# MartinMikkelsen/TensorTrainNumerics.jl

Hardware: AMD Instinct MI355X
Metric: TT cores/sec for QTT Laplacian apply+round, d=30 rank-64 (higher is better)
Workload: dtype f64

## Files before the change

### tensortrainnumerics.jl_amd/csrc/ttn_dense_kernels.h

```cpp
#pragma once
#include "ttn_wg_prims.h"
#include "ttn_wg_gemm.h"
#include "ttn_wg_lq.h"
#include "ttn_wg_jacobi.h"
#include "ttn_wg_chol.h"

struct CompressArgs {
    TTDev tt;
    long long max_bond;
    double truncerr;
    int sweeps;
    int k_single;
    int k_first, k_last;
    double* scratch;
    long long scratch_stride;
    int pmax, qmax;
    double* sv_out;
    int sv_steps;
    int* status;
    int* sweep_stats;
    int fast;
    int fused;
    TTODev op;
    TTDev x;
// ... 739 lines not shown
            for (int kk = wave; kk < half; kk += TTN_NWAVES) {
                int i, j;
                if (kk == 0) { i = round; j = pe - 1; }
                else { i = (round + kk) % (pe - 1); j = (round + pe - 1 - kk) % (pe - 1); }
                if (i > j) { const int t = i; i = j; j = t; }
                if (j >= p) continue;
                lds_f64* xi = Ms + i * LDQ;
                lds_f64* xj = Ms + j * LDQ;
                double u[4], v[4];
                double a = 0.0, b_ = 0.0, g = 0.0;
#pragma unroll
                for (int t4 = 0; t4 < 4; ++t4) {
                    const int c = lane + 64 * t4;
                    u[t4] = (c < q) ? xi[c] : 0.0; v[t4] = (c < q) ? xj[c] : 0.0;
                    a = fma(u[t4], u[t4], a); b_ = fma(v[t4], v[t4], b_); g = fma(u[t4], v[t4], g);
                }
                a = wave_sum(a); b_ = wave_sum(b_); g = wave_sum(g);
                if (a <= aneg || b_ <= aneg) continue;
                if (g * g <= tol2 * a * b_) continue;
                const double dd = b_ - a, hh = g + g;
                const double hyp = __builtin_amdgcn_sqrt(fma(dd, dd, hh * hh));
                const double t = copysign(hh * __builtin_amdgcn_rcp(fabs(dd) + hyp), hh * dd);
                const double cs = fast_rsqrt2(fma(t, t, 1.0)), sn = cs * t;
#pragma unroll
                for (int t4 = 0; t4 < 4; ++t4) {
                    const int c = lane + 64 * t4;
                    if (c < q) { xi[c] = cs * u[t4] - sn * v[t4]; xj[c] = sn * u[t4] + cs * v[t4]; }
                }
                if (lane < p) { const double u = Es[i * 17 + lane], v = Es[j * 17 + lane]; Es[i * 17 + lane] = cs * u - sn * v; Es[j * 17 + lane] = sn * u + cs * v; }
                rotated = 1;
            }
            __syncthreads();
        }
        if (rotated && lane == 0) atomicOr((int*)flg, 1);
        __syncthreads();
        conv = !(*flg);
        __syncthreads();
    }
    for (int i = wave; i < p; i += TTN_NWAVES) {
        double a = 0.0;
        for (int j = lane; j < q; j += 64) { const double v = Ms[i * LDQ + j]; a = fma(v, v, a); }
        a = wave_sum(a);
        if (lane == 0) nr[i] = sqrt(a);
    }
    __syncthreads();
    for (int c = tid; c < p; c += TTN_WG) {
        const double sc = nr[c];
        int pos = 0;
        for (int j = 0; j < p; ++j) { const double sj = nr[j]; pos += (sj > sc) || (sj == sc && j < c); }
        Q.perm[pos] = c;
        Q.sigs[pos] = sc;
    }
    __syncthreads();
    const int r = wg_rank_rule_core(Q.rank_rule, Q.truncerr, Q.max_bond, Q.sigs, Q.iflag, p, p, s0);
    if (Q.sv_row)
        for (int i = tid; i < Q.pmax; i += TTN_WG) Q.sv_row[i] = (i < p) ? Q.sigs[i] * s0 : -1.0;
    const View Lfv = mkview(ck, Idx{Dl, (long long)n1, 1}, plain((long long)n1 * Dl));
    const View Rfv = mkview(ck1, plain(n2), Idx{n2, 1, (long long)n2 * r});
    const View Lo = wide ? Lfv : tview(Rfv);
    const View Ro = wide ? Rfv : tview(Lfv);
    const double sq0 = sqrt(s0);
    for (int e = tid; e < p * r; e += TTN_WG) {
        const int row = e % p, j = e / p;
        const double sj = Q.sigs[j];
        const int pj = Q.perm[j];
        const bool keep = (sj > 0.0) && (sj * sj > aneg);
        Lo.p[ix(Lo.r, row) + ix(Lo.c, j)] = keep ? Es[pj * 17 + row] * (sq0 * sqrt(sj)) : 0.0;
    }
    for (int e = tid; e < r * q; e += TTN_WG) {
        const int col = e % q, j = e / q;
        const double sj = Q.sigs[j];
        const int pj = Q.perm[j];
        const bool keep = (sj > 0.0) && (sj * sj > aneg);
        Ro.p[ix(Ro.r, j) + ix(Ro.c, col)] = keep ? Ms[pj * LDQ + col] * (sq0 / sqrt(sj)) : 0.0;
    }
    if (tid == 0) { *rank_out = r; if (!conv) *Q.status_b = TTN_ST_JACOBI; }
    __syncthreads();
    return sweeps;
}

__device__ int wg_eig128(const double* Gg, double* Vst, int r, int nev, double* sig, double* lds, int* iwork, double* dwork);
__device__ int wg_eig64(const double* Gg, int ldg, double* Vst, int r, int nev, double* sig, double* lds, int* iwork, double* dwork);

struct BondIO {
    double *ck, *ck1;
    int n1, n2, Dl, rm, Dr;
    long long* rank_out;
    int cap;
};
template <int SWAP>
__device__ __forceinline__ void wg_bond_step_io(const CompressArgs& P, int b, const BondIO& io, int k, int step, double* lds, bool virt) {
    const int tid = threadIdx.x;
    const int n1 = io.n1, n2 = io.n2;
    const int Dl = io.Dl, rm = io.rm, Dr = io.Dr;
    const int mr = n1 * Dl, mc = n2 * Dr;
    double* ck = io.ck;
    double* ck1 = io.ck1;
    const View Am = mkview(ck, Idx{Dl, (long long)n1, 1}, plain((long long)n1 * Dl));
    const View Bm = mkview(ck1, plain(n2), Idx{n2, 1, (long long)n2 * rm});
    const bool wide = mr <= mc;
    const int p = wide ? mr : mc, q = wide ? mc : mr;
    const View Ap = wide ? Am : tview(Bm);
    const View Bp = wide ? Bm : tview(Am);

    BondCtx S;
    S.ldsX = lds;
    S.red = lds + GEMM_LDS_TOTAL;
    S.Ts = S.red + 32;
    S.Ss = S.Ts + QR_NB * QR_NB;
    S.taus = S.Ss + QR_NB * QR_NB;
    S.scal = S.taus + QR_NB;
    S.iflag = reinterpret_cast<int*>(S.scal + 8);
    S.nrm2 = S.scal + 16;
    double* scr = P.scratch + (long long)blockIdx.x * P.scratch_stride;
    const long long pq = (long long)P.pmax * P.qmax;
    S.M = scr;
    S.M2 = S.M + pq;
    S.Vb = S.M2 + pq;
    S.Wb = S.Vb + (long long)QR_NB * P.qmax;
    S.Us = S.Wb + (long long)P.pmax * QR_NB;
    S.Xg = S.Us + (long long)P.pmax * P.pmax;
    S.sig = S.Xg + (long long)P.pmax * P.pmax;
    S.sigs = S.sig + P.pmax;
    S.perm = reinterpret_cast<int*>(S.sigs + P.pmax);
    S.Ga = S.sigs + 2 * P.pmax;
    S.Gb = S.Ga + 128 * 128;
    S.Cc = S.Gb + 128 * 128;
    S.T1 = S.Cc + 128 * 128;
    S.T2 = S.T1 + 128 * 128;
    S.T3 = S.T2 + 128 * 128;
    if (pq >= 3 * 128 * 128) {
        S.Ga = S.M2; S.Gb = S.M2 + 128 * 128; S.T2 = S.M2 + 2 * 128 * 128;
    }

    bool virt_live = false;
    if (virt) {
        if (wide && rm >= p) virt_live = true;
        else wg_materialize_core(P, b, k + 1);
    }

    const View Lfv = mkview(ck, Idx{Dl, (long long)n1, 1}, plain((long long)n1 * Dl));
    int nsw_total = 0;
    bool done = false;

    if (SWAP == 0 && P.fast && rm < p && rm <= TTN_LDS_COLS && rm >= 2) {
        double sa = 0.0, sb = 0.0;
        sa = wg_absmax(ck, (long long)n1 * Dl * rm, S.red);
        sb = wg_absmax(ck1, (long long)n2 * rm * Dr, S.red);
        bool ok = (sa > 0.0) && (sb > 0.0);
        const double sA = wide ? sa : sb, sB = wide ? sb : sa;
        const double s0 = sA * sB;
        const View Gav = mkview(S.Ga, plain(1), plain(128));
        const View Gbv = mkview(S.Gb, plain(1), plain(128));
        const View Ccv = mkview(S.Cc, plain(1), plain(128));
        bool diagA = false;
        if (ok) {
            wg_syrk2(rm, p, tview(Ap), Gav, 1.0 / (sA * sA), rm, q, Bp, Gbv, 1.0 / (sB * sB), lds);
            if (rm == 64 && !(P.fast & 4) && !(P.fast & 8)) {
                const double wmax = wg_diag_test_t3(S.Ga, S.Gb, S.T3, S.Ss, S.red);
                diagA = wmax <= FAST_DIAG_TOL;
            }
            if (diagA) {
            } else if (rm <= TTN_LDS_COLS / 2) {
                for (int e = tid; e < rm * 128; e += TTN_WG) if ((e & 127) < rm) { S.ldsX[e] = S.Ga[e]; S.ldsX[TTN_LDS_IMG / 2 + e] = S.Gb[e]; }
                __syncthreads();
                ok = wg_chol2_lds128(rm, S.ldsX, S.Ts, S.iflag, S.scal + 1) == 0;
                for (int e = tid; e < rm * 128; e += TTN_WG) if ((e & 127) < rm) { S.Ga[e] = S.ldsX[e]; S.Gb[e] = S.ldsX[TTN_LDS_IMG / 2 + e]; }
                __syncthreads();
            } else {
                for (int e = tid; e < rm * 128; e += TTN_WG) if ((e & 127) < rm) S.ldsX[e] = S.Ga[e];
                __syncthreads();
                ok = wg_chol_lds128(rm, S.ldsX, S.red, S.iflag, S.scal + 1) == 0;
                for (int e = tid; e < rm * 128; e += TTN_WG) if ((e & 127) < rm) S.Ga[e] = S.ldsX[e];
                __syncthreads();
                if (ok) {
                    for (int e = tid; e < rm * 128; e += TTN_WG) if ((e & 127) < rm) S.ldsX[e] = S.Gb[e];
                    __syncthreads();
                    ok = wg_chol_lds128(rm, S.ldsX, S.red, S.iflag, S.scal + 1) == 0;
                    for (int e = tid; e < rm * 128; e += TTN_WG) if ((e & 127) < rm) S.Gb[e] = S.ldsX[e];
                    __syncthreads();
                }
            }
        }
        int r = 0, rk = 0;
        if (ok) {
            int nsw = 1;
            if (diagA) {
                ok = wg_eig64(S.T3, 128, S.T2, 64, 64, S.sigs, lds, reinterpret_cast<int*>(S.Ts), S.Ts + 64) == 0;
                for (int j = tid; j < 64; j += TTN_WG) S.perm[j] = j;
                if (tid == 0) S.scal[0] = 64.0 * DBL_EPSILON * DBL_EPSILON * S.sigs[0] * S.sigs[0];
                __syncthreads();
            } else {
            wg_gemm(rm, rm, rm, tview(Gav), Gbv, Ccv, 1.0, 0.0, lds);
            if (rm == 64 && !(P.fast & 4)) {
                wg_gemm(64, 64, 64, Ccv, tview(Ccv), mkview(S.T3, plain(1), plain(128)), 1.0, 0.0, lds);
                ok = wg_eig64(S.T3, 128, S.T2, 64, 64, S.sigs, lds, reinterpret_cast<int*>(S.Ts), S.Ts + 64) == 0;
                for (int j = tid; j < 64; j += TTN_WG) S.perm[j] = j;
                if (tid == 0) S.scal[0] = 64.0 * DBL_EPSILON * DBL_EPSILON * S.sigs[0] * S.sigs[0];
                __syncthreads();
            } else {
                for (int e = tid; e < rm * 128; e += TTN_WG) { const int c = e >> 7, r_ = e & 127; S.ldsX[e] = (r_ < rm) ? S.Cc[c * 128 + r_] : 0.0; }
                __syncthreads();
                nsw = uni32(wg_svd_cols(P, S, rm, S.ldsX, 128, true));
                nsw_total += (nsw < 0 ? -nsw : nsw);
            }
            }
            ok = ok && (nsw > 0) && (S.sigs[rm - 1] * FAST_KAPPA_MAX >= S.sigs[0]) && (S.sigs[rm - 1] * S.sigs[rm - 1] > S.scal[0]);
        }
        if (ok) {
            r = wg_rank_rule(P, S, rm, p, s0);
            rk = r < rm ? r : rm;
            const double fa = sqrt(s0) / sA, fb = sqrt(s0) / sB;
            if (diagA) {
                wg_scale_t12_diag(S.ldsX, S.sigs, S.perm, S.Ga, S.T1, S.T2, rk, fa, fb, S.Ts);
            } else {
                for (int e = tid; e < rm * rk; e += TTN_WG) {
                    const int row = e % rm, j = e / rm;
                    const double sj = S.sigs[j], xv = S.ldsX[S.perm[j] * 128 + row];
                    const double rs = sqrt(sj);
                    S.T1[j * 128 + row] = xv * (fa / (sj * sj * rs));
                    S.T2[j * 128 + row] = xv * (fb / (sj * rs));
                }
                __syncthreads();
            }
            const View T1v = mkview(S.T1, plain(1), plain(128));
            const View T2v = mkview(S.T2, plain(1), plain(128));
            double* LfT = S.M;
            double* RfT = S.M + (long long)p * rk;
            const View Lft = mkview(LfT, plain(1), plain(p));
            const View Rft = mkview(RfT, plain(q), plain(1));
            if (diagA) {
                wg_gemm_ra2(rk, p, rm, tview(T1v), tview(Ap), tview(Lft), 1.0, rk, q, rm, tview(T2v), Bp, Rft, 1.0, lds);
            } else {
            wg_gemm(rm, rk, rm, tview(Ccv), T1v, mkview(S.T3, plain(1), plain(128)), 1.0, 0.0, lds);
            wg_gemm(rm, rk, rm, Gbv, mkview(S.T3, plain(1), plain(128)), T1v, 1.0, 0.0, lds);
            wg_gemm(p, rk, rm, Ap, T1v, Lft, 1.0, 0.0, lds);
            wg_gemm(rm, rk, rm, Gav, T2v, mkview(S.T3, plain(1), plain(128)), 1.0, 0.0, lds);
            wg_gemm(rk, q, rm, tview(mkview(S.T3, plain(1), plain(128))), Bp, Rft, 1.0, 0.0, lds);
            }
            wg_syrk2(rk, p, tview(Lft), mkview(S.T1, plain(1), plain(128)), 1.0, rk, q, Rft, mkview(S.T2, plain(1), plain(128)), 1.0, lds);
            ok = wg_check_diag_tab2(S.sigs, S.T1, S.T2, 128, rk, s0, S.Ts, S.red) <= FAST_CHECK_TOL;
            if (ok) {
                if (P.sv_out && step < P.sv_steps) {
                    double* so = P.sv_out + ((long long)b * P.sv_steps + step) * P.pmax;
                    for (int i = tid; i < P.pmax; i += TTN_WG) so[i] = (i < rm) ? S.sigs[i] * s0 : (i < p ? 0.0 : -1.0);
                }
                const View Rfv = mkview(ck1, plain(n2), Idx{n2, 1, (long long)n2 * r});
                const View Lo = wide ? Lfv : tview(Rfv);
                const View Ro = wide ? Rfv : tview(Lfv);
                __syncthreads();
                wg_copy_to_view(Lo, LfT, p, r, 1, p, rk, 1);
                wg_copy_to_view(Ro, RfT, r, q, q, 1, rk, 0);
                if (tid == 0) *io.rank_out = r;
                __syncthreads();
                done = true;
            }
        }
    }

    if (!done) {
        const View Mv = mkview(S.M, plain(q), plain(1));
        bool merged = false;
        if (virt_live) {
            merged = wg_fused_merge(P, b, k, p, q, Am, S.M, S.M2, pq, lds, S.scal + 6, S.red);
            if (!merged) wg_materialize_core(P, b, k + 1);
        }
        double mx_swap = 0.0;
        if (SWAP != 0) {
            for (int sA = 0; sA < n1; ++sA)
                for (int sB = 0; sB < n2; ++sB) {
                    const View Av = mkview(ck + sA, plain(n1), plain((long long)n1 * Dl));
                    const View Bv = mkview(ck1 + sB, plain(n2), plain((long long)n2 * rm));
                    if (wide) wg_gemm(Dl, Dr, rm, Av, Bv, mkview(S.M + (long long)Dl * sB * q + sA, plain(q), plain(n1)), 1.0, 0.0, lds, S.scal + 6);
                    else wg_gemm(Dr, Dl, rm, tview(Bv), tview(Av), mkview(S.M + (long long)sA * q + (long long)Dl * sB, plain((long long)n1 * q), plain(1)), 1.0, 0.0, lds, S.scal + 6);
                    mx_swap = fmax(mx_swap, unif64(S.scal[6]));
                    __syncthreads();
                }
        } else if (!merged) wg_gemm(p, q, rm, Ap, Bp, Mv, 1.0, 0.0, lds, S.scal + 6);
        const double mx = (SWAP != 0) ? mx_swap : unif64(S.scal[6]);
        const double s0 = (mx > 0.0) ? mx : 1.0;
        const double inv_s0 = 1.0 / s0;
        const bool need_lq = q > p;
        const bool x_in_lds = p <= TTN_LDS_COLS;
        double* X = x_in_lds ? S.ldsX : S.Xg;
        int ldx = x_in_lds ? 128 : p;

        const bool lq_in_lds = (long long)p * q <= GEMM_LDS_DOUBLES || GEMM_LDS_DOUBLES / p >= 2 * p;
        const bool eig_ok = SWAP == 0 && P.fast && !(P.fast & 2) && need_lq && ((p > 64 && p <= 128 && P.max_bond <= 64) || (p == 64 && P.max_bond < 64));
        const bool cholqr_ok = SWAP == 0 && P.fast && need_lq && x_in_lds && p >= 16 && p <= 64 && (long long)p * q > GEMM_LDS_DOUBLES;
        for (int attempt = (SWAP == 0 && P.fast && need_lq && (eig_ok || cholqr_ok || (x_in_lds && !lq_in_lds)) && p >= 2) ? 1 : 2; attempt <= 2 && !done; ++attempt) {
            bool ok = true;
            bool use_eig = false;
            bool cholqr = false;
            double gram_trace = 0.0;
            X = (x_in_lds || attempt == 1) ? S.ldsX : S.Xg;
            ldx = (x_in_lds || attempt == 1) ? 128 : p;
            if (attempt == 1) {
                wg_syrk(p, q, Mv, mkview(S.Ga, plain(1), plain(128)), inv_s0 * inv_s0, lds);
                use_eig = eig_ok;
                if (use_eig) {
                    if (p > 64 && p < 128) {
                        for (int e = tid; e < 128 * 128; e += TTN_WG)
                            if ((e & 127) >= p || (e >> 7) >= p) S.Ga[e] = 0.0;
                        __syncthreads();
                    }
                    const int r0 = (int)P.max_bond;
                    const int nev = (P.truncerr > 0.0 || (P.sv_out && step < P.sv_steps)) ? p : r0;
                    { double t_ = 0.0; for (int i = tid; i < p; i += TTN_WG) t_ += S.Ga[i * 129]; gram_trace = unif64(wg_sum(t_, S.red)); }
                    ok = ((p == 64) ? wg_eig64(S.Ga, 128, S.Gb, r0, nev, S.sigs, lds, reinterpret_cast<int*>(S.Ts), S.Ts + 64)
                                    : wg_eig128(S.Ga, S.Gb, r0, nev, S.sigs, lds, reinterpret_cast<int*>(S.Ts), S.Ts + 64)) == 0;
                    for (int j = tid; j < p; j += TTN_WG) { S.perm[j] = j; if (j >= nev) S.sigs[j] = 0.0; }
                    if (tid == 0) S.scal[0] = (double)p * DBL_EPSILON * DBL_EPSILON * S.sigs[0] * S.sigs[0];
                    __syncthreads();
                } else {
                wg_img_load(S.ldsX, 0, S.Ga, p, S.red);
                ok = wg_chol_lds128(p, S.ldsX, S.red, S.iflag, S.scal + 1) == 0;
                if (ok && (P.truncerr > 0.0 || (long long)p <= P.max_bond)) {
                    if (cholqr_ok) { if (unif64(S.scal[1]) <= CHOLQR_PIVOT_MAX) cholqr = true; else ok = false; }
                    else if (unif64(S.scal[1]) > FAST_KAPPA_MAX * FAST_KAPPA_MAX) ok = false;
                }
                if (cholqr) {
                    for (int e = tid; e < p * p; e += TTN_WG) { const int i = e % p, j = e / p; S.T1[i + 128 * j] = S.ldsX[i + 128 * j]; }
                    wg_trsm_lower_cols(p, q, S.ldsX, S.M, q, inv_s0, S.M2, q);
                    const View Q1v = mkview(S.M2, plain(q), plain(1));
                    wg_syrk(p, q, Q1v, mkview(S.Cc, plain(1), plain(128)), 1.0, lds);
                    const double dev = wg_img_load(S.ldsX, 0, S.Cc, p, S.red);
                    ok = dev <= CHOLQR_ORTH_MAX && wg_chol_lds128(p, S.ldsX, S.red, S.iflag, S.scal + 1) == 0;
                    if (ok) {
                        wg_img_load(S.ldsX, 64, S.T1, p, S.red);
                        wg_tril_mul_lds(p, S.ldsX);
                    }
                }
                for (int e = tid; e < p * 128; e += TTN_WG) if ((e & 127) >= p) S.ldsX[e] = 0.0;
                __syncthreads();
                }
            } else {
                if (need_lq) {
                    wg_copy_scale(S.M2, S.M, (long long)p * q, inv_s0);
                    __syncthreads();
                    wg_lq_blocked(p, q, S.M2, q, S.Vb, S.Wb, nullptr, nullptr, lds, S.Ts, S.Ss, S.taus, S.red);
                }
                const double* Lsrc = need_lq ? S.M2 : S.M;
                if (need_lq && x_in_lds) {
// ... 59 lines not shown
                    wg_gemm_ra(r, q, p, mkview(S.Us, plain(p), plain(1)), Mv, mkview(S.M2, plain(q), plain(1)), inv_s0, lds);
                    for (int e = tid; e < r * 128; e += TTN_WG) { const int c = e & 127, j = e >> 7; S.ldsX[e] = (c < q) ? S.M2[(long long)j * q + c] : 0.0; }
                    __syncthreads();
                    const int nsp = uni32(wg_svd_cols(P, S, r, S.ldsX, 128, true, q));
                    nsw_total += (nsp < 0 ? -nsp : nsp);
                    if (nsp <= 0) continue;
                    const View Rfv = mkview(ck1, plain(n2), Idx{n2, 1, (long long)n2 * r});
                    const View Lo = wide ? Lfv : tview(Rfv);
                    const View Ro = wide ? Rfv : tview(Lfv);
                    const double sq0 = sqrt(s0), aneg = S.scal[0];
                    for (int e = tid; e < r * q; e += TTN_WG) {
                        const int col = e % q, j = e / q;
                        const double sj = S.sigs[j], xv = S.ldsX[S.perm[j] * 128 + col];
                        const bool keep = (sj > 0.0) && (sj * sj > aneg);
                        Ro.p[ix(Ro.r, j) + ix(Ro.c, col)] = keep ? xv * (sq0 / sqrt(sj)) : 0.0;
                        S.M2[(long long)j * q + col] = keep ? xv * (sq0 / (sj * sqrt(sj))) : 0.0;
                    }
                    __syncthreads();
                    wg_gemm(p, r, q, Mv, mkview(S.M2, plain(1), plain(q)), Lo, inv_s0, 0.0, lds);
                    if (P.sv_out && step < P.sv_steps) {
                        double* so = P.sv_out + ((long long)b * P.sv_steps + step) * P.pmax;
                        for (int i = tid; i < P.pmax; i += TTN_WG) so[i] = (i < p) ? S.sigs[i] * s0 : -1.0;
                    }
                    if (tid == 0) *io.rank_out = r;
                    __syncthreads();
                    done = true;
                    continue;
                }
            }
            if (attempt == 2 && P.sv_out && step < P.sv_steps) {
                double* so = P.sv_out + ((long long)b * P.sv_steps + step) * P.pmax;
                for (int i = tid; i < P.pmax; i += TTN_WG) so[i] = (i < p) ? S.sigs[i] * s0 : -1.0;
            }
            const View Rfv = mkview(ck1, plain(n2), Idx{n2, 1, (long long)n2 * r});
            const View Lo = wide ? Lfv : tview(Rfv);
            const View Ro = wide ? Rfv : tview(Lfv);
            const double sq0 = sqrt(s0);
            const double aneg = S.scal[0];
            if (p <= 128 && r <= 128) {
                wg_scale_image(X, ldx, (x_in_lds || attempt == 1) ? 1 : 0, S.sigs, S.perm, Lo, S.Us, p, r, s0, aneg, (SWAP == 0) ? 0 : (wide ? 1 : 2), S.Ts);
            } else {
            for (int e = tid; e < p * r; e += TTN_WG) {
                const int row = e % p, j = e / p;
                const double sj = S.sigs[j];
                const double xv = X[(long long)S.perm[j] * ldx + row];
                const bool keep = (sj > 0.0) && (sj * sj > aneg);
                double lf, us;
                if (SWAP == 0) { lf = keep ? xv * (sq0 / sqrt(sj)) : 0.0; us = keep ? xv * (sq0 / (sj * sqrt(sj))) : 0.0; }
                else if (wide) { lf = keep ? xv / sj : 0.0; us = keep ? xv * (s0 / sj) : 0.0; }
                else { lf = keep ? xv * s0 : 0.0; us = keep ? xv / (sj * sj) : 0.0; }
                Lo.p[ix(Lo.r, row) + ix(Lo.c, j)] = lf;
                S.Us[(long long)j * p + row] = us;
            }
            }
            __syncthreads();
            wg_gemm_ra(r, q, p, mkview(S.Us, plain(p), plain(1)), Mv, Ro, inv_s0, lds);
            if (attempt == 1) {
                wg_syrk(r, q, Ro, mkview(S.T2, plain(1), plain(128)), 1.0, lds);
                const double e2 = (r <= 128) ? wg_check_diag_tab(S.sigs, S.T2, 128, r, s0, S.Ts, S.red) : unif64(wg_check_diag(S, S.T2, 128, r, s0));
                if (!(e2 <= (cholqr ? CHOLQR_CHECK_TOL : FAST_CHECK_TOL))) continue;
                if (P.sv_out && step < P.sv_steps) {
                    double* so = P.sv_out + ((long long)b * P.sv_steps + step) * P.pmax;
                    for (int i = tid; i < P.pmax; i += TTN_WG) so[i] = (i < p) ? S.sigs[i] * s0 : -1.0;
                }
            }
            if (tid == 0) *io.rank_out = r;
            __syncthreads();
            done = true;
        }
    }
    if (tid == 0) P.sweep_stats[b] += nsw_total;
    __syncthreads();
}

__device__ __forceinline__ void wg_bond_step(const CompressArgs& P, int b, int k, int step, double* lds, bool virt = false ) {
    const TTDev& T = P.tt;
    long long* rks = T.rks + (long long)b * (T.d + 1);
    BondIO io;
    io.n1 = uni32(T.dims[k]); io.n2 = uni32(T.dims[k + 1]);
    io.Dl = uni32((int)rks[k]); io.rm = uni32((int)rks[k + 1]); io.Dr = uni32((int)rks[k + 2]);
    io.ck = T.data + (long long)b * T.stride + T.off[k];
    io.ck1 = T.data + (long long)b * T.stride + T.off[k + 1];
    io.rank_out = rks + k + 1;
    {
        const int mr = io.n1 * io.Dl, mc = io.n2 * io.Dr;
        const int p = mr <= mc ? mr : mc, q = mr <= mc ? mc : mr;
        if (P.fast && p >= 2 && p <= SMALL_STEP_PMAX && q <= SMALL_STEP_QMAX && P.pmax >= p) {
            if (virt) wg_materialize_core(P, b, k + 1);
            SmallStepArgs Q;
            Q.truncerr = P.truncerr; Q.max_bond = P.max_bond; Q.rank_rule = P.rank_rule; Q.pmax = P.pmax;
            Q.sv_row = (P.sv_out && step < P.sv_steps) ? P.sv_out + ((long long)b * P.sv_steps + step) * P.pmax : nullptr;
            Q.status_b = P.status + b;
            Q.red = lds + GEMM_LDS_TOTAL;
            Q.scal = Q.red + 32 + 2 * QR_NB * QR_NB + QR_NB;
            Q.iflag = reinterpret_cast<int*>(Q.scal + 8);
            double* scr = P.scratch + (long long)blockIdx.x * P.scratch_stride;
            const long long pq = (long long)P.pmax * P.qmax;
            double* sig = scr + 2 * pq + (long long)QR_NB * P.qmax + (long long)P.pmax * QR_NB + 2LL * P.pmax * P.pmax;
            Q.sigs = sig + P.pmax;
            Q.perm = reinterpret_cast<int*>(Q.sigs + P.pmax);
            const int nsw = wg_bond_small(Q, io.ck, io.ck1, io.n1, io.n2, io.Dl, io.rm, io.Dr, io.rank_out, lds);
            if (threadIdx.x == 0) P.sweep_stats[b] += nsw;
            __syncthreads();
            return;
        }
    }
    wg_bond_step_io<0>(P, b, io, k, step, lds, virt);
}

__global__ void TTN_KERNEL_BOUNDS k_compress(CompressArgs P) {
    TTN_SETPRIO_BASE();
    extern __shared__ double lds[];
    const int d = P.tt.d;
    const int per_sweep = 2 * (d - 1);
    const int nsteps = (P.k_single > 0) ? 1 : (P.k_single < 0) ? ((P.k_first <= P.k_last ? P.k_last - P.k_first : P.k_first - P.k_last) + 1)
                                                               : P.sweeps * per_sweep;
    int b = blockIdx.x;
    while (b < P.tt.batch) {
        if (threadIdx.x == 0) P.sweep_stats[b] = 0;
        __syncthreads();
        if (P.fused && !(P.k_single < 0 && P.fused_first_real)) wg_materialize_core(P, b, (P.k_single < 0) ? P.k_first : 0);
        for (int step = 0; step < nsteps; ++step) {
            int k;
            bool virt = false;
            if (P.k_single > 0) k = P.k_single - 1;
            else if (P.k_single < 0) { k = (P.k_first <= P.k_last) ? P.k_first + step : P.k_first - step; virt = P.fused != 0; }
            else {
                const int i = step % per_sweep;
                k = (i < d - 1) ? i : per_sweep - 1 - i;
                virt = P.fused && step < d - 1;
            }
            wg_bond_step(P, b, k, step, lds, virt);
        }
        if (!P.next_train) break;
        int* nb = reinterpret_cast<int*>(lds + GEMM_LDS_TOTAL);
        if (threadIdx.x == 0) *nb = (int)gridDim.x + atomicAdd(P.next_train, 1);
        __syncthreads();
        b = uni32(*nb);
        __syncthreads();
    }
}
```

### tensortrainnumerics.jl_amd/csrc/ttn_wg_gemm.h

```cpp
#pragma once
#include "ttn_wg_prims.h"

#define GEMM_BK 16
#define GEMM_LD 145
#define GEMM_LDS_DOUBLES (TTN_LDS_IMG + 512)


struct GemmDesc {
    int m, n, k, pad;
    View A, B, C;
    double alpha, beta;
    unsigned long long* amax;
};
#if TTN_WG == 512
#define GEMM_TAB_ENTRIES 704
#define GEMM_KSLAB 512
#define GEMM_SMALL_KMAX 256
#else
#define GEMM_TAB_ENTRIES 1536
#define GEMM_KSLAB 768
#define GEMM_SMALL_KMAX 512
#endif
#define GEMM_DESC_DOUBLES (32 + GEMM_TAB_ENTRIES)
#define GEMM_LDS_TOTAL (GEMM_LDS_DOUBLES + GEMM_DESC_DOUBLES)
// ... 418 lines not shown
                const int kk = (K0) + fx + 16 * u;                                                                      \
                co_[u] = colT[kk < q ? kk : 0];                                                                         \
            }                                                                                                           \
            _Pragma("unroll") for (int j = 0; j < JMAX; ++j) {                                                           \
                const int row = sy + RG * j;                                                                            \
                _Pragma("unroll") for (int u = 0; u < KC16; ++u) {                                                       \
                    const int kk = (K0) + fx + 16 * u;                                                                  \
                    v[j][u] = Ag[(row < p && kk < q) ? ro[j] + co_[u] : 0];                                             \
                }                                                                                                       \
            }                                                                                                           \
        }
        SYRK_LOAD(0)
        for (int k0 = 0; k0 < qall; k0 += KC) {
#pragma unroll
            for (int j = 0; j < JMAX; ++j) {
                const int row = sy + RG * j;
#pragma unroll
                for (int u = 0; u < KC16; ++u) {
                    const int kl = fx + 16 * u;
                    if (row < pp) Cs[kl * LD + row] = (row < p && k0 + kl < q) ? v[j][u] : 0.0;
                }
            }
            __syncthreads();
            if (k0 + KC < q) { SYRK_LOAD(k0 + KC) }
            const int ksteps = (q - k0 < KC) ? (q - k0 + 3) >> 2 : KC / 4;
            if constexpr (NT > 0) {
                if (TEAMS == 1 || ksteps > 0) syrk_ksteps<NT, LD, KC / 4>(acc, Cs + lk * LD + li, ksteps, ta, tb);
            }
            __syncthreads();
        }
#undef SYRK_LOAD
#pragma unroll
        for (int u = 0; u < NT; ++u) res[u] = acc[u];
    };
    if (nlive == MAXT) body(syrk_nt<MAXT>{});
    else if (MAXT > 1 && nlive == MAXT - 1) body(syrk_nt<(MAXT > 1 ? MAXT - 1 : 0)>{});
    else if (MAXT > 2 && nlive == MAXT - 2) body(syrk_nt<(MAXT > 2 ? MAXT - 2 : 0)>{});
    else if (MAXT > 3 && nlive == MAXT - 3) body(syrk_nt<(MAXT > 3 ? MAXT - 3 : 0)>{});
    else if (MAXT > 4 && nlive == MAXT - 4) body(syrk_nt<(MAXT > 4 ? MAXT - 4 : 0)>{});
    else body(syrk_nt<0>{});
    static_assert(MAXT <= 5, "one copy of the body per number of live tiles");
#pragma unroll
    for (int u = 0; u < MAXT; ++u) {
        if (u >= nlive) continue;
#pragma unroll
        for (int reg = 0; reg < 4; ++reg) {
            const int gi = 16 * t_r[u] + lk + 4 * reg, gj = 16 * t_c[u] + li;
            if (gi < p && gj < p) {
                const double val = alpha * res[u][reg];
                Cg[ix(C.r, gi) + ix(C.c, gj)] = val;
                if (t_r[u] != t_c[u]) Cg[ix(C.r, gj) + ix(C.c, gi)] = val;
            }
        }
    }
    __syncthreads();
}
template <int KC16, int JMAX, int MAXT>
__device__ __noinline__ void wg_syrk_impl(const GemmDesc* dsc_, double* lds) { syrk_body<KC16, JMAX, MAXT, 1>(dsc_, lds); }
__device__ __noinline__ void wg_syrk2_impl(const GemmDesc* dsc_, double* lds) {
#if TTN_WG == 512
    syrk_body<3, 4, 3, 2>(dsc_, lds);
#else
    syrk_body<3, 2, 2, 2>(dsc_, lds);
#endif
}

__device__ inline void wg_syrk(int p, int q, View A, View G, double alpha, double* lds) {
    if (p > 128 || q > SYRK_QMAX) { wg_gemm(p, p, q, A, tview(A), G, alpha, 0.0, lds); return; }
    GemmDesc* dsc = reinterpret_cast<GemmDesc*>(lds + GEMM_LDS_DOUBLES);
    __syncthreads();
    if (threadIdx.x == 0) { dsc->m = p; dsc->n = p; dsc->k = q; dsc->pad = 0; dsc->A = A; dsc->C = G; dsc->alpha = alpha; dsc->beta = 0.0; dsc->amax = nullptr; }
    __syncthreads();
    TTN_SETPRIO_GEMM();
#if TTN_WG == 512
    if (p > 64) wg_syrk_impl<3, 4, 5>(dsc, lds);
    else wg_syrk_impl<6, 2, 2>(dsc, lds);
#else
    if (p > 64) wg_syrk_impl<6, 2, 3>(dsc, lds);
    else wg_syrk_impl<6, 1, 1>(dsc, lds);
#endif
    TTN_SETPRIO_BASE();
}

__device__ inline void wg_syrk2(int p1, int q1, View A1, View G1, double alpha1, int p2, int q2, View A2, View G2, double alpha2, double* lds) {
    if (p1 > 64 || p2 > 64 || q1 > SYRK2_QMAX || q2 > SYRK2_QMAX) {
        wg_syrk(p1, q1, A1, G1, alpha1, lds);
        wg_syrk(p2, q2, A2, G2, alpha2, lds);
        return;
    }
    GemmDesc* dsc = reinterpret_cast<GemmDesc*>(lds + GEMM_LDS_DOUBLES);
    static_assert(2 * sizeof(GemmDesc) <= 64 * sizeof(double), "two descriptors in front of the two-team tables");
    __syncthreads();
    if (threadIdx.x == 0) {
        dsc[0].m = p1; dsc[0].n = p1; dsc[0].k = q1; dsc[0].pad = 0; dsc[0].A = A1; dsc[0].C = G1; dsc[0].alpha = alpha1; dsc[0].beta = 0.0; dsc[0].amax = nullptr;
        dsc[1].m = p2; dsc[1].n = p2; dsc[1].k = q2; dsc[1].pad = 0; dsc[1].A = A2; dsc[1].C = G2; dsc[1].alpha = alpha2; dsc[1].beta = 0.0; dsc[1].amax = nullptr;
    }
    __syncthreads();
    TTN_SETPRIO_GEMM();
    wg_syrk2_impl(dsc, lds);
    TTN_SETPRIO_BASE();
}

#define GEMM_RA_NMAX (2 * GEMM_TAB_ENTRIES - 320)
#define RA_RING 3
template <int NB, int LD>
__device__ __forceinline__ mfma_acc_t ra_ksteps(const double* areg, const lds_f64* bp) {
    mfma_acc_t acc = (mfma_acc_t){0.0, 0.0, 0.0, 0.0};
    double b[RA_RING];
#pragma unroll
    for (int t = 0; t < RA_RING; ++t) b[t] = bp[4 * t * LD];
    __builtin_amdgcn_sched_barrier(0);
#pragma unroll
    for (int ks = 0; ks < 8 * NB; ++ks) {
        acc = __builtin_amdgcn_mfma_f64_16x16x4f64(areg[ks], b[ks % RA_RING], acc, 0, 0, 0);
        if (ks + RA_RING < 8 * NB) b[ks % RA_RING] = bp[4 * (ks + RA_RING) * LD];
        __builtin_amdgcn_sched_barrier(0);
    }
    return acc;
}
__device__ __noinline__ void wg_gemm_ra_impl(const GemmDesc* dsc_, double* lds) {
    const lds_gdesc* dsc = (const lds_gdesc*)dsc_;
    constexpr int CG = TTN_NWAVES / 4, NC = 16 * CG;
    constexpr int LD = (NC == 32) ? 49 : 81;
    constexpr int KR = 128 / (TTN_WG / NC);
    static_assert(128 * LD <= GEMM_LDS_DOUBLES, "a chunk holds all of k");
    const int m = uni32(dsc->m), n = uni32(dsc->n), k = uni32(dsc->k);
    const View A = ldsView(&dsc->A), B = ldsView(&dsc->B), C = ldsView(&dsc->C);
    const double alpha = unif64(dsc->alpha);
    const int tid = threadIdx.x, lane = tid & 63, wave = tid >> 6;
    const int li = lane & 15, lk = lane >> 4;
    const int rt = uni32(wave & 3), cg = uni32(wave >> 2);
    lds_f64* Bs = (lds_f64*)lds;
    lds_i32* rowA = (lds_i32*)(lds + GEMM_LDS_DOUBLES + 32);
    lds_i32* kA = rowA + 64;
    lds_i32* kB = kA + 128;
    lds_i32* colB = kB + 128;
    for (int i = tid; i < 64; i += TTN_WG) rowA[i] = (i < m) ? (int)ix(A.r, i) : 0;
    for (int i = tid; i < 128; i += TTN_WG) { kA[i] = (i < k) ? (int)ix(A.c, i) : 0; kB[i] = (i < k) ? (int)ix(B.r, i) : 0; }
    for (int i = tid; i < n; i += TTN_WG) colB[i] = (int)ix(B.c, i);
    __syncthreads();
    gmem_f64* Ag = (gmem_f64*)A.p;
    gmem_f64* Bg = (gmem_f64*)B.p;
    gmem_wf64* Cg = (gmem_wf64*)C.p;
    const int ksteps = (k + 3) >> 2;
    double areg[32];
    {
        const int row = rt * 16 + li, ro = rowA[row < 64 ? row : 0];
#pragma unroll
        for (int ks = 0; ks < 32; ++ks) {
            const int kk = 4 * ks + lk, ka = kA[kk];
            areg[ks] = Ag[(row < m && kk < k) ? ro + ka : 0];
        }
#pragma unroll
        for (int ks = 0; ks < 32; ++ks) { const int kk = 4 * ks + lk; if (!(row < m && kk < k)) areg[ks] = 0.0; }
    }
    const int fx = tid % NC, sy = tid / NC;
    double v[KR];
#define RA_LOAD(C0)                                                                                                     \
    {                                                                                                                   \
        const int col = (C0) + fx;                                                                                      \
        const int co = colB[col < n ? col : 0];                                                                         \
        int kb_[KR];                                                                                                    \
        _Pragma("unroll") for (int u = 0; u < KR; ++u) kb_[u] = kB[sy + (TTN_WG / NC) * u];                             \
        _Pragma("unroll") for (int u = 0; u < KR; ++u) {                                                                 \
            const int kk = sy + (TTN_WG / NC) * u;                                                                      \
            v[u] = Bg[(col < n && kk < k) ? co + kb_[u] : 0];                                                           \
        }                                                                                                               \
    }
    RA_LOAD(0)
    const bool live = rt * 16 < m;
    const int nb = uni32((ksteps + 7) >> 3);
    for (int c0 = 0; c0 < n; c0 += NC) {
#pragma unroll
        for (int u = 0; u < KR; ++u) {
            const int kk = sy + (TTN_WG / NC) * u;
            Bs[kk * LD + fx] = (c0 + fx < n && kk < k) ? v[u] : 0.0;
        }
        __syncthreads();
// ... 37 lines not shown
    constexpr int TWG = TTN_WG / 2, NC = 32, LD = 49, KMAX = 64;
    constexpr int KR = KMAX / (TWG / NC);
    static_assert(TWG == 256 && 2 * KMAX * LD <= GEMM_LDS_DOUBLES, "one chunk per team holds all of k");
    const int team = uni32((int)threadIdx.x / TWG);
    const lds_gdesc* dsc = (const lds_gdesc*)dsc_ + team;
    const int m = uni32(dsc->m), n = uni32(dsc->n), k = uni32(dsc->k);
    const int no = uni32(((const lds_gdesc*)dsc_ + (1 - team))->n), nall = n > no ? n : no;
    const View A = ldsView(&dsc->A), B = ldsView(&dsc->B), C = ldsView(&dsc->C);
    const double alpha = unif64(dsc->alpha);
    const int tid = threadIdx.x - team * TWG, lane = tid & 63;
    const int li = lane & 15, lk = lane >> 4;
    const int rt = uni32(tid >> 6);
    lds_f64* Bs = (lds_f64*)lds + team * (KMAX * LD);
    lds_i32* rowA = (lds_i32*)(lds + GEMM_LDS_DOUBLES + 64) + team * SYRK2_TAB;
    lds_i32* kA = rowA + 64;
    lds_i32* kB = kA + KMAX;
    lds_i32* colB = kB + KMAX;
    for (int i = tid; i < 64; i += TWG) {
        rowA[i] = (i < m) ? (int)ix(A.r, i) : 0;
        kA[i] = (i < k) ? (int)ix(A.c, i) : 0;
        kB[i] = (i < k) ? (int)ix(B.r, i) : 0;
    }
    for (int i = tid; i < n; i += TWG) colB[i] = (int)ix(B.c, i);
    __syncthreads();
    gmem_f64* Ag = (gmem_f64*)A.p;
    gmem_f64* Bg = (gmem_f64*)B.p;
    gmem_wf64* Cg = (gmem_wf64*)C.p;
    double areg[KMAX / 4];
    {
        const int row = rt * 16 + li, ro = rowA[row];
#pragma unroll
        for (int ks = 0; ks < KMAX / 4; ++ks) {
            const int kk = 4 * ks + lk, ka = kA[kk];
            areg[ks] = Ag[(row < m && kk < k) ? ro + ka : 0];
        }
#pragma unroll
        for (int ks = 0; ks < KMAX / 4; ++ks) { const int kk = 4 * ks + lk; if (!(row < m && kk < k)) areg[ks] = 0.0; }
    }
    const int fx = tid % NC, sy = tid / NC;
    double v[KR];
#define RA2_LOAD(C0)         \
    {                                                                                                                   \
        const int col = (C0) + fx;                                                                                      \
        const int co = colB[col < n ? col : 0];                                                                         \
        int kb_[KR];                                                                                                    \
        _Pragma("unroll") for (int u = 0; u < KR; ++u) kb_[u] = kB[sy + (TWG / NC) * u];                                \
        _Pragma("unroll") for (int u = 0; u < KR; ++u) {                                                                 \
            const int kk = sy + (TWG / NC) * u;                                                                         \
            v[u] = Bg[(col < n && kk < k) ? co + kb_[u] : 0];                                                           \
        }                                                                                                               \
    }
    RA2_LOAD(0)
    const bool live = rt * 16 < m;
    const int nb = uni32((((k + 3) >> 2) + 7) >> 3);
    for (int c0 = 0; c0 < nall; c0 += NC) {
#pragma unroll
        for (int u = 0; u < KR; ++u) {
            const int kk = sy + (TWG / NC) * u;
            Bs[kk * LD + fx] = (c0 + fx < n && kk < k) ? v[u] : 0.0;
        }
        __syncthreads();
        if (c0 + NC < n) RA2_LOAD(c0 + NC)
#pragma unroll
        for (int cg = 0; cg < 2; ++cg) {
            if (live && c0 + cg * 16 < n) {
                const lds_f64* bp = Bs + lk * LD + cg * 16 + li;
                mfma_acc_t acc;
                if (nb == 2) acc = ra_ksteps<2, LD>(areg, bp);
                else acc = ra_ksteps<1, LD>(areg, bp);
#pragma unroll
                for (int reg = 0; reg < 4; ++reg) {
                    const int gi = rt * 16 + lk + 4 * reg, gj = c0 + cg * 16 + li;
                    if (gi < m && gj < n) Cg[ix(C.r, gi) + ix(C.c, gj)] = alpha * acc[reg];
                }
            }
        }
        __syncthreads();
    }
#undef RA2_LOAD
}
#endif

__device__ inline void wg_gemm_ra2(int m1, int n1, int k1, View A1, View B1, View C1, double alpha1,
                                   int m2, int n2, int k2, View A2, View B2, View C2, double alpha2, double* lds) {
#if TTN_WG == 512
    if (m1 <= 64 && m2 <= 64 && k1 <= 64 && k2 <= 64 && n1 >= 64 && n2 >= 64 && n1 <= GEMM_RA2_NMAX && n2 <= GEMM_RA2_NMAX) {
        GemmDesc* dsc = reinterpret_cast<GemmDesc*>(lds + GEMM_LDS_DOUBLES);
        __syncthreads();
        if (threadIdx.x == 0) {
            dsc[0].m = m1; dsc[0].n = n1; dsc[0].k = k1; dsc[0].pad = 0; dsc[0].A = A1; dsc[0].B = B1; dsc[0].C = C1; dsc[0].alpha = alpha1; dsc[0].beta = 0.0; dsc[0].amax = nullptr;
            dsc[1].m = m2; dsc[1].n = n2; dsc[1].k = k2; dsc[1].pad = 0; dsc[1].A = A2; dsc[1].B = B2; dsc[1].C = C2; dsc[1].alpha = alpha2; dsc[1].beta = 0.0; dsc[1].amax = nullptr;
        }
        __syncthreads();
        TTN_SETPRIO_GEMM();
        wg_gemm_ra2_impl(dsc, lds);
        TTN_SETPRIO_BASE();
        return;
    }
#endif
    wg_gemm_ra(m1, n1, k1, A1, B1, C1, alpha1, lds);
    wg_gemm_ra(m2, n2, k2, A2, B2, C2, alpha2, lds);
}
```

Before: 679,400.

## Hand over truncated bond factors through scratch between consecutive sweep steps

Adds a handover mechanism. During the backward half of a rounding sweep, the left factor of a bond step stays in the workgroup's scratch staging area and is not written back to the core in global memory. The next step then reads that staged matrix directly as its B operand for the absmax, syrk and gemm calls. Write-back copies are skipped when the rank is unchanged, and the staged data is restored to the core whenever the following step cannot consume it. This is meant to cut global memory round-trips and copy passes per bond step, at the cost of considerable bookkeeping complexity, extra view indirection through LDS, and a risk of correctness bugs.

```diff
diff --git a/tensortrainnumerics.jl_amd/csrc/ttn_dense_kernels.h b/tensortrainnumerics.jl_amd/csrc/ttn_dense_kernels.h
--- a/tensortrainnumerics.jl_amd/csrc/ttn_dense_kernels.h
+++ b/tensortrainnumerics.jl_amd/csrc/ttn_dense_kernels.h
@@ -845,6 +845,31 @@
 __device__ int wg_eig128(const double* Gg, double* Vst, int r, int nev, double* sig, double* lds, int* iwork, double* dwork);
 __device__ int wg_eig64(const double* Gg, int ldg, double* Vst, int r, int nev, double* sig, double* lds, int* iwork, double* dwork);
 
+__device__ inline long long handover_area(const CompressArgs& P) { return (long long)P.pmax * P.qmax / 3; }
+__device__ inline bool handover_fits(const CompressArgs& P, int p, int q, int rm) {
+    const long long h = handover_area(P);
+    return (long long)p * rm <= h && (long long)rm * q <= h;
+}
+__device__ inline bool handover_next(const CompressArgs& P, int step) {
+    if (P.k_single > 0) return false;
+    if (P.k_single < 0) return P.k_first > P.k_last && step < P.k_first - P.k_last && !P.fused;
+    const int d = P.tt.d, i = step % (2 * (d - 1));
+    return i >= d - 1 && i + 1 < 2 * (d - 1);
+}
+__device__ inline int* handover_note(const CompressArgs& P) {
+    double* scr = P.scratch + (long long)blockIdx.x * P.scratch_stride;
+    const long long pq = (long long)P.pmax * P.qmax;
+    double* sigs = scr + 2 * pq + (long long)QR_NB * P.qmax + (long long)P.pmax * QR_NB + 2LL * P.pmax * P.pmax + P.pmax;
+    return reinterpret_cast<int*>(sigs + P.pmax) + P.pmax;
+}
+__device__ __noinline__ void wg_handover_restore(double* core, const double* stage, int n2, int rm, int Dr, int* note) {
+    core = unip(core); stage = unip(stage); n2 = uni32(n2); rm = uni32(rm); Dr = uni32(Dr); note = unip(note);
+    __syncthreads();
+    wg_copy_to_view(mkview(core, Idx{rm, (long long)n2, 1}, plain((long long)n2 * rm)), stage, n2 * rm, Dr, 1, (long long)n2 * rm, Dr, 1);
+    if (threadIdx.x == 0) *note = 0;
+    __syncthreads();
+}
+
 struct BondIO {
     double *ck, *ck1;
     int n1, n2, Dl, rm, Dr;
@@ -909,7 +934,10 @@
     if (SWAP == 0 && P.fast && rm < p && rm <= TTN_LDS_COLS && rm >= 2) {
         double sa = 0.0, sb = 0.0;
         sa = wg_absmax(ck, (long long)n1 * Dl * rm, S.red);
-        sb = wg_absmax(ck1, (long long)n2 * rm * Dr, S.red);
+#define HANDOVER_PEND() ((SWAP == 0) ? uni32(*handover_note(P)) : 0)
+#define HANDOVER_BS(pn) mkview(S.M + ((pn) == 2 ? handover_area(P) : 0), plain(1), plain(rm))
+#define HANDOVER_B(pn) ((pn) ? HANDOVER_BS(pn) : Bp)
+        { const int pn = HANDOVER_PEND(); sb = wg_absmax(pn ? S.M + (pn == 2 ? handover_area(P) : 0) : ck1, (long long)n2 * rm * Dr, S.red); }
         bool ok = (sa > 0.0) && (sb > 0.0);
         const double sA = wide ? sa : sb, sB = wide ? sb : sa;
         const double s0 = sA * sB;
@@ -918,7 +946,7 @@
         const View Ccv = mkview(S.Cc, plain(1), plain(128));
         bool diagA = false;
         if (ok) {
-            wg_syrk2(rm, p, tview(Ap), Gav, 1.0 / (sA * sA), rm, q, Bp, Gbv, 1.0 / (sB * sB), lds);
+            { const int pn = HANDOVER_PEND(); wg_syrk2(rm, p, tview(Ap), Gav, 1.0 / (sA * sA), rm, q, Bp, Gbv, 1.0 / (sB * sB), lds, pn, HANDOVER_BS(pn)); }
             if (rm == 64 && !(P.fast & 4) && !(P.fast & 8)) {
                 const double wmax = wg_diag_test_t3(S.Ga, S.Gb, S.T3, S.Ss, S.red);
                 diagA = wmax <= FAST_DIAG_TOL;
@@ -988,21 +1016,31 @@
             }
             const View T1v = mkview(S.T1, plain(1), plain(128));
             const View T2v = mkview(S.T2, plain(1), plain(128));
-            double* LfT = S.M;
-            double* RfT = S.M + (long long)p * rk;
-            const View Lft = mkview(LfT, plain(1), plain(p));
-            const View Rft = mkview(RfT, plain(q), plain(1));
+#define HANDOVER_LFT(pn) (S.M + ((pn) == 1 ? handover_area(P) : 0))
+#define HANDOVER_RFT(pn) ((pn) ? S.M + 2 * handover_area(P) : S.M + (long long)p * rk)
+#define HANDOVER_RFS(pn) mkview(HANDOVER_RFT(pn), plain(q), plain(1))
+#define HANDOVER_RFC() mkview(ck1, plain(n2), Idx{n2, 1, (long long)n2 * r})
+#define HANDOVER_RF(pn) (((pn) && rk == r) ? HANDOVER_RFC() : HANDOVER_RFS(pn))
+            const int pn = HANDOVER_PEND();
+            const View Lft = mkview(HANDOVER_LFT(pn), plain(1), plain(p));
+            const View Rft = HANDOVER_RF(pn);
+            View* hv = reinterpret_cast<View*>(S.taus);
+            static_assert(2 * sizeof(View) <= QR_NB * sizeof(double), "two views in S.taus");
+            if (tid == 0) { hv[0] = HANDOVER_B(pn); hv[1] = Rft; }
             if (diagA) {
-                wg_gemm_ra2(rk, p, rm, tview(T1v), tview(Ap), tview(Lft), 1.0, rk, q, rm, tview(T2v), Bp, Rft, 1.0, lds);
+                wg_gemm_ra2(rk, p, rm, tview(T1v), tview(Ap), tview(Lft), 1.0, rk, q, rm, tview(T2v), Bp, mkview(S.M + (long long)p * rk, plain(q), plain(1)), 1.0, lds, hv);
             } else {
             wg_gemm(rm, rk, rm, tview(Ccv), T1v, mkview(S.T3, plain(1), plain(128)), 1.0, 0.0, lds);
             wg_gemm(rm, rk, rm, Gbv, mkview(S.T3, plain(1), plain(128)), T1v, 1.0, 0.0, lds);
             wg_gemm(p, rk, rm, Ap, T1v, Lft, 1.0, 0.0, lds);
             wg_gemm(rm, rk, rm, Gav, T2v, mkview(S.T3, plain(1), plain(128)), 1.0, 0.0, lds);
-            wg_gemm(rk, q, rm, tview(mkview(S.T3, plain(1), plain(128))), Bp, Rft, 1.0, 0.0, lds);
-            }
-            wg_syrk2(rk, p, tview(Lft), mkview(S.T1, plain(1), plain(128)), 1.0, rk, q, Rft, mkview(S.T2, plain(1), plain(128)), 1.0, lds);
+            wg_gemm(rk, q, rm, tview(mkview(S.T3, plain(1), plain(128))), HANDOVER_B(pn), Rft, 1.0, 0.0, lds);
+            }
+            { const int pc = HANDOVER_PEND();
+              wg_syrk2(rk, p, tview(mkview(HANDOVER_LFT(pc), plain(1), plain(p))), mkview(S.T1, plain(1), plain(128)), 1.0, rk, q, mkview(S.M + (long long)p * rk, plain(q), plain(1)), mkview(S.T2, plain(1), plain(128)), 1.0, lds,
+                       0, View{}, reinterpret_cast<const View*>(S.taus) + 1); }
             ok = wg_check_diag_tab2(S.sigs, S.T1, S.T2, 128, rk, s0, S.Ts, S.red) <= FAST_CHECK_TOL;
+            if ((P.fast & 32) && HANDOVER_PEND()) ok = false;
             if (ok) {
                 if (P.sv_out && step < P.sv_steps) {
                     double* so = P.sv_out + ((long long)b * P.sv_steps + step) * P.pmax;
@@ -1011,10 +1049,12 @@
                 const View Rfv = mkview(ck1, plain(n2), Idx{n2, 1, (long long)n2 * r});
                 const View Lo = wide ? Lfv : tview(Rfv);
                 const View Ro = wide ? Rfv : tview(Lfv);
+                const bool hand = SWAP == 0 && wide && rk == r && handover_next(P, step);
+                const int pc = HANDOVER_PEND();
                 __syncthreads();
-                wg_copy_to_view(Lo, LfT, p, r, 1, p, rk, 1);
-                wg_copy_to_view(Ro, RfT, r, q, q, 1, rk, 0);
-                if (tid == 0) *io.rank_out = r;
+                if (!hand) wg_copy_to_view(Lo, HANDOVER_LFT(pc), p, r, 1, p, rk, 1);
+                if (!(pc && rk == r)) wg_copy_to_view(Ro, HANDOVER_RFT(pc), r, q, q, 1, rk, 0);
+                if (tid == 0) { *io.rank_out = r; if (pc || hand) *handover_note(P) = hand ? (pc == 1 ? 2 : 1) : 0; }
                 __syncthreads();
                 done = true;
             }
@@ -1022,6 +1062,21 @@
     }
 
     if (!done) {
+        if (const int pn = HANDOVER_PEND()) {
+            const double* stage = S.M + (pn == 2 ? handover_area(P) : 0);
+            __syncthreads();
+            for (int e = tid; e < n2 * rm * Dr; e += TTN_WG) { const int s2 = e % n2, ga = (e / n2) % rm, be = e / (n2 * rm); ck1[e] = stage[ga + rm * s2 + n2 * rm * be]; }
+            if (tid == 0) *handover_note(P) = 0;
+            __syncthreads();
+        }
+#undef HANDOVER_PEND
+#undef HANDOVER_B
+#undef HANDOVER_BS
+#undef HANDOVER_RFS
+#undef HANDOVER_RFC
+#undef HANDOVER_LFT
+#undef HANDOVER_RFT
+#undef HANDOVER_RF
         const View Mv = mkview(S.M, plain(q), plain(1));
         bool merged = false;
         if (virt_live) {
@@ -1247,10 +1302,17 @@
     io.ck = T.data + (long long)b * T.stride + T.off[k];
     io.ck1 = T.data + (long long)b * T.stride + T.off[k + 1];
     io.rank_out = rks + k + 1;
+    const int mr = io.n1 * io.Dl, mc = io.n2 * io.Dr;
+    const int p = mr <= mc ? mr : mc, q = mr <= mc ? mc : mr;
+    const bool small = P.fast && p >= 2 && p <= SMALL_STEP_PMAX && q <= SMALL_STEP_QMAX && P.pmax >= p;
+    int pend = uni32(*handover_note(P));
     {
-        const int mr = io.n1 * io.Dl, mc = io.n2 * io.Dr;
-        const int p = mr <= mc ? mr : mc, q = mr <= mc ? mc : mr;
-        if (P.fast && p >= 2 && p <= SMALL_STEP_PMAX && q <= SMALL_STEP_QMAX && P.pmax >= p) {
+        const bool take = !small && !virt && P.fast && mr <= mc && io.rm < p && io.rm <= TTN_LDS_COLS && io.rm >= 2 && handover_fits(P, p, q, io.rm);
+        if (pend && !take) {
+            wg_handover_restore(io.ck1, P.scratch + (long long)blockIdx.x * P.scratch_stride + (pend == 2 ? handover_area(P) : 0), io.n2, io.rm, io.Dr, handover_note(P));
+            pend = 0;
+        }
+        if (small) {
             if (virt) wg_materialize_core(P, b, k + 1);
             SmallStepArgs Q;
             Q.truncerr = P.truncerr; Q.max_bond = P.max_bond; Q.rank_rule = P.rank_rule; Q.pmax = P.pmax;
@@ -1282,7 +1344,7 @@
                                                                : P.sweeps * per_sweep;
     int b = blockIdx.x;
     while (b < P.tt.batch) {
-        if (threadIdx.x == 0) P.sweep_stats[b] = 0;
+        if (threadIdx.x == 0) { P.sweep_stats[b] = 0; *handover_note(P) = 0; }
         __syncthreads();
         if (P.fused && !(P.k_single < 0 && P.fused_first_real)) wg_materialize_core(P, b, (P.k_single < 0) ? P.k_first : 0);
         for (int step = 0; step < nsteps; ++step) {
diff --git a/tensortrainnumerics.jl_amd/csrc/ttn_wg_gemm.h b/tensortrainnumerics.jl_amd/csrc/ttn_wg_gemm.h
--- a/tensortrainnumerics.jl_amd/csrc/ttn_wg_gemm.h
+++ b/tensortrainnumerics.jl_amd/csrc/ttn_wg_gemm.h
@@ -524,8 +524,11 @@
     TTN_SETPRIO_BASE();
 }
 
-__device__ inline void wg_syrk2(int p1, int q1, View A1, View G1, double alpha1, int p2, int q2, View A2, View G2, double alpha2, double* lds) {
+__device__ inline void wg_syrk2(int p1, int q1, View A1, View G1, double alpha1, int p2, int q2, View A2, View G2, double alpha2, double* lds,
+                                int alt2 = 0, View A2alt = View{}, const View* ovr2 = nullptr) {
     if (p1 > 64 || p2 > 64 || q1 > SYRK2_QMAX || q2 > SYRK2_QMAX) {
+        if (alt2) A2 = A2alt;
+        if (ovr2) { __syncthreads(); A2 = uniView(*ovr2); }
         wg_syrk(p1, q1, A1, G1, alpha1, lds);
         wg_syrk(p2, q2, A2, G2, alpha2, lds);
         return;
@@ -536,6 +539,8 @@
     if (threadIdx.x == 0) {
         dsc[0].m = p1; dsc[0].n = p1; dsc[0].k = q1; dsc[0].pad = 0; dsc[0].A = A1; dsc[0].C = G1; dsc[0].alpha = alpha1; dsc[0].beta = 0.0; dsc[0].amax = nullptr;
         dsc[1].m = p2; dsc[1].n = p2; dsc[1].k = q2; dsc[1].pad = 0; dsc[1].A = A2; dsc[1].C = G2; dsc[1].alpha = alpha2; dsc[1].beta = 0.0; dsc[1].amax = nullptr;
+        if (alt2) dsc[1].A = A2alt;
+        if (ovr2) dsc[1].A = *ovr2;
     }
     __syncthreads();
     TTN_SETPRIO_GEMM();
@@ -739,7 +744,7 @@
 #endif
 
 __device__ inline void wg_gemm_ra2(int m1, int n1, int k1, View A1, View B1, View C1, double alpha1,
-                                   int m2, int n2, int k2, View A2, View B2, View C2, double alpha2, double* lds) {
+                                   int m2, int n2, int k2, View A2, View B2, View C2, double alpha2, double* lds, const View* ovr2 = nullptr) {
 #if TTN_WG == 512
     if (m1 <= 64 && m2 <= 64 && k1 <= 64 && k2 <= 64 && n1 >= 64 && n2 >= 64 && n1 <= GEMM_RA2_NMAX && n2 <= GEMM_RA2_NMAX) {
         GemmDesc* dsc = reinterpret_cast<GemmDesc*>(lds + GEMM_LDS_DOUBLES);
@@ -747,6 +752,7 @@
         if (threadIdx.x == 0) {
             dsc[0].m = m1; dsc[0].n = n1; dsc[0].k = k1; dsc[0].pad = 0; dsc[0].A = A1; dsc[0].B = B1; dsc[0].C = C1; dsc[0].alpha = alpha1; dsc[0].beta = 0.0; dsc[0].amax = nullptr;
             dsc[1].m = m2; dsc[1].n = n2; dsc[1].k = k2; dsc[1].pad = 0; dsc[1].A = A2; dsc[1].B = B2; dsc[1].C = C2; dsc[1].alpha = alpha2; dsc[1].beta = 0.0; dsc[1].amax = nullptr;
+            if (ovr2) { dsc[1].B = ovr2[0]; dsc[1].C = ovr2[1]; }
         }
         __syncthreads();
         TTN_SETPRIO_GEMM();
@@ -756,5 +762,6 @@
     }
 #endif
     wg_gemm_ra(m1, n1, k1, A1, B1, C1, alpha1, lds);
+    if (ovr2) { __syncthreads(); B2 = uniView(ovr2[0]); C2 = uniView(ovr2[1]); }
     wg_gemm_ra(m2, n2, k2, A2, B2, C2, alpha2, lds);
 }
```

Result: faster. 687,000, median of 6 (+1.1%).
